# sanje2v/DualSuperResLearningForSemSeg

Hardware: AMD Instinct MI355X
Metric: stage-3 train images/sec at 256x512->512x1024 (higher is better)
Workload: dtype f32; 1 GPU; DSRL stage 3 (ResNet-101 OS16 + ASPP + SSSR/SISR decoders + FA loss), full train step, random-init weights, 256x512 input -> 512x1024 logits; global_batch=8, per_gpu_batch=8, parallelism=dp1, optimizer=SGD m0.9 wd5e-4 lr0.006

## Files before the change

dualsuperreslearningforsemseg_amd/_lib.py:

```python
import ctypes as C
import os

import torch

_HERE = os.path.dirname(os.path.abspath(__file__))
LIB_PATH = os.path.join(_HERE, 'libdsrl_hip.so')

fp = C.c_void_p
i32 = C.c_int
i64 = C.c_int64
u64 = C.c_uint64
u32 = C.c_uint32
f32 = C.c_float
sz = C.c_size_t
stream_t = C.c_void_p

_conv_shape = [i32] * 10


class WgradProblem(C.Structure):
    _fields_ = [('x', C.c_void_p), ('dy', C.c_void_p), ('dw', C.c_void_p)] + [(n, C.c_int32) for n in
                ('ldx', 'lddy', 'N', 'H', 'W', 'C', 'K', 'R', 'S', 'stride', 'pad', 'dil')] + [('x_amax', C.c_void_p), ('dy_amax', C.c_void_p)]


PROTOTYPES = {
    'dsrl_version': (i32, []),
    'dsrl_last_error': (C.c_char_p, []),
    'dsrl_device_check': (i32, [C.POINTER(i32)]),
    'dsrl_conv2d_fwd_workspace_bytes': (sz, _conv_shape),
    'dsrl_conv2d_fwd': (i32, [fp, i32, fp, fp, fp, i32] + _conv_shape + [fp, sz, stream_t]),
    'dsrl_conv2d_fwd_stats_parts': (i32, _conv_shape),
    'dsrl_conv2d_fwd_stats': (i32, [fp, i32, fp, fp, fp, i32] + _conv_shape + [fp, sz, fp, i32, stream_t]),
    'dsrl_conv2d_dgrad_workspace_bytes': (sz, _conv_shape),
    'dsrl_conv2d_transposed_filter_floats': (sz, [i32] * 4),
    'dsrl_conv2d_transpose_filter': (i32, [fp, fp, i32, i32, i32, i32, stream_t]),
    'dsrl_conv2d_transpose_filters_batched': (i32, [fp, i32, i64, stream_t]),
    'dsrl_conv2d_filters_amax_segment_floats': (i32, []),
    'dsrl_conv2d_filters_amax_batched': (i32, [fp, i64, stream_t]),
    'dsrl_conv2d_dgrad': (i32, [fp, i32, fp, fp, fp, i32] + _conv_shape + [fp, sz, stream_t]),
    'dsrl_conv2d_dgrad_stats_parts': (i32, _conv_shape),
    'dsrl_conv2d_dgrad_bnstats': (i32, [fp, i32, fp, fp, fp, i32] + _conv_shape + [fp, sz, fp, i32, fp, i32, fp, fp, i32, fp, i32, i32, stream_t]),
    'dsrl_conv2d_dgrad_accumulate': (i32, [fp, i32, fp, fp, fp, i32] + _conv_shape + [fp, sz, stream_t]),
    'dsrl_conv2d_wgrad_workspace_bytes': (sz, _conv_shape),
    'dsrl_conv2d_wgrad': (i32, [fp, i32, fp, i32, fp] + _conv_shape + [fp, sz, stream_t]),
    'dsrl_conv2d_wgrad_group_table_bytes': (sz, [i32]),
    'dsrl_conv2d_wgrad_group_workspace_bytes': (sz, [fp, i32]),
    'dsrl_conv2d_wgrad_group_plan': (i32, [fp, i32, fp, sz, fp, fp, sz]),
    'dsrl_conv2d_wgrad_group_launch': (i32, [fp, fp, stream_t]),
    'dsrl_amax': (i32, [fp, i32, i64, i32, fp, stream_t]),
    'dsrl_conv2d_fwd_amax': (i32, [fp, i32, fp, fp, fp, fp, fp, fp, i32] + _conv_shape + [fp, sz, fp, i32, stream_t]),
    'dsrl_conv2d_dgrad_amax': (i32, [fp, i32, fp, fp, fp, fp, fp, fp, i32] + _conv_shape + [fp, sz, fp, i32, fp, i32, fp, fp, i32, fp, i32, i32, stream_t]),
    'dsrl_conv2d_split_filters_batched': (i32, [fp, i32, i64, stream_t]),
    'dsrl_planes_lo_offset': (sz, [i64]),
    'dsrl_planes_bytes': (sz, [i64, i32]),
    'dsrl_split_planes': (i32, [fp, i32, i64, i32, fp, fp, i32, stream_t]),
    'dsrl_conv2d_filter_planes_batched': (i32, [fp, i32, i64, stream_t]),
    'dsrl_conv2d_fwd_planes': (i32, [fp, i32, fp, fp, fp, fp, fp, fp, fp, fp, i32] + _conv_shape + [fp, sz, fp, i32, stream_t]),
    'dsrl_conv2d_dgrad_planes': (i32, [fp, i32, fp, fp, fp, fp, fp, fp, fp, fp, i32] + _conv_shape + [fp, sz, fp, i32, fp, i32, fp, fp, i32, fp, i32, i32, stream_t]),
    'dsrl_conv2d_dgrad_planes_drop': (i32, [fp, i32, fp, fp, fp, fp, fp, fp, fp, fp, i32] + _conv_shape + [fp, sz, fp, i32, fp, i32, fp, fp, i32, f32, fp, i32, i32, stream_t]),
    'dsrl_conv2d_wgrad_amax': (i32, [fp, i32, fp, fp, i32, fp, fp] + _conv_shape + [fp, sz, stream_t]),
    'dsrl_conv_precision': (i32, [i32]),
    'dsrl_conv2d_inbounds_macs': (i64, _conv_shape),
    'dsrl_conv2d_rowfold_fwd_workspace_bytes': (sz, [i32] * 9),
    'dsrl_conv2d_rowfold_fwd': (i32, [fp, i32, fp, fp, fp, i32] + [i32] * 9 + [i64, fp, sz, stream_t]),
    'dsrl_conv2d_rowfold_wgrad_workspace_bytes': (sz, [i32] * 9),
    'dsrl_conv2d_rowfold_wgrad': (i32, [fp, i32, fp, i32, fp] + [i32] * 9 + [i64, fp, sz, stream_t]),
    'dsrl_pad_image_nhwc': (i32, [fp, i64, i64, i64, i64, fp] + [i32] * 9 + [stream_t]),
    'dsrl_colsum_workspace_bytes': (sz, [i64, i32]),
    'dsrl_colsum': (i32, [fp, i32, i64, i32, fp, fp, sz, stream_t]),
    'dsrl_bn_workspace_bytes': (sz, [i64, i32]),
# ... 122 lines not shown
```

dualsuperreslearningforsemseg_amd/command_handlers/train_or_resume.py:

```python
import glob
import os
from datetime import datetime

import torch as t
import torch.distributed as dist

from .. import functional as HF
from .. import settings
from ..ddp import FlatParams
from ..models import DSRL
from ..models.losses import FALoss


def isCUDAdevice(device):
    return device.casefold() == 'gpu'


def polynomial_lr(base_lr, end_lr, epoch, max_decay_steps, power):
    if epoch <= 0:
        return base_lr
    return (base_lr - end_lr) * ((1. - epoch / max_decay_steps) ** power) + end_lr


class SyntheticCityscapes:
# ... 139 lines not shown

    def _set_hyper(self, hp):
        vals = (float(hp[0]), float(hp[1]), float(hp[2]), 1.0 / self.flat.world)
        if vals != self._hyper_vals:
            self._hyper_host.copy_(t.tensor(vals, dtype=t.float32))
            self.hyper.copy_(self._hyper_host, non_blocking=True)
            self._hyper_vals = vals

    def _graph_key(self, input_image, input_org, target):
        return (tuple(input_image.shape), tuple(input_org.shape), tuple(target.shape), HF.get_conv_precision(), HF.overlap_wgrad)

    def _capture(self, key, input_image, input_org, target, hp):
        c = _CapturedStep()
        c.img, c.org, c.tgt = input_image.clone(), input_org.clone(), target.clone()
        bns = [m for m in self.model.modules() if isinstance(m, t.nn.modules.batchnorm._BatchNorm)]
        before = [getattr(m, '_dsrl_batches', 0) for m in bns]
        step_before = HF._rng_state['step']
        c.graph = t.cuda.CUDAGraph()
        overlap_was = HF.overlap_wgrad
        HF.overlap_wgrad = False
        c.keep = HF.graph_keepalive = []
        HF.capture_host, HF.capture_host_off = t.empty(2 << 20, dtype=t.uint8, pin_memory=True), 0
        c.keep.append(HF.capture_host)
        if HF.f16_mode():
            c.keep.append(HF.amax_pin(self.flat.device))
        c.graph_b, c.ready = None, []
        mode = 'thread_local'
        try:
            if self.split:
                with t.cuda.graph(c.graph, capture_error_mode=mode):
                    c.outs, c.vals, cuts = self._phase_a(c.img, c.org, c.tgt, True, True, True)
                c.ready = self.flat.ready_chunks()
                c.graph_b = t.cuda.CUDAGraph()
                with t.cuda.graph(c.graph_b, pool=c.graph.pool(), capture_error_mode=mode):
                    self._phase_b(cuts)
                del cuts
            else:
                with t.cuda.graph(c.graph, capture_error_mode=mode):
                    c.outs, c.vals, _ = self._phase_a(c.img, c.org, c.tgt, True, True, False)
                    self._finish(hp, True)
        finally:
            HF.overlap_wgrad = overlap_was
            HF.graph_keepalive = None
            HF.capture_host = None
        HF._rng_state['step'] = step_before
        c.bns = [m for m, n in zip(bns, before) if getattr(m, '_dsrl_batches', 0) != n]
        for m, n in zip(bns, before):
            if hasattr(m, '_dsrl_batches'):
                m._dsrl_batches = n
        self._graphs[key] = c
        return c

    def _capture_or_fall_back(self, key, input_image, input_org, target, hp):
        import sys
        bns = [m for m in self.model.modules() if isinstance(m, t.nn.modules.batchnorm._BatchNorm)]
        before = [getattr(m, '_dsrl_batches', 0) for m in bns]
        step_before, overlap_was = HF._rng_state['step'], HF.overlap_wgrad
        try:
            return self._capture(key, input_image, input_org, target, hp)
        except Exception as e:
            print(f'[dsrl] hipGraph capture failed ({type(e).__name__}: {str(e)[:200]}); this TrainStep continues with eager launches', file=sys.stderr, flush=True)
            self.use_graph = False
            HF.overlap_wgrad, HF.graph_keepalive, HF.capture_host, HF.wgrad_queue = overlap_was, None, None, None
            HF._rng_state['step'] = step_before
            for m, n in zip(bns, before):
                if hasattr(m, '_dsrl_batches'):
                    m._dsrl_batches = n
            try:
                t.cuda.set_stream(t.cuda.default_stream(self.flat.device))
                t.cuda.synchronize(self.flat.device)
            except Exception:
                pass
            return None

    def _replay(self, c, input_image, input_org, target):
        flat = self.flat
        for dst, src in ((c.img, input_image), (c.org, input_org), (c.tgt, target)):
            if dst.data_ptr() != src.data_ptr():
                dst.copy_(src, non_blocking=True)
        ev = [t.cuda.Event(enable_timing=True) for _ in range(4)] if (self.time_collectives and flat.world > 1) else None
        if flat.world > 1:
            if ev:
                ev[0].record()
            flat.sync_buffers()
            if ev:
                ev[1].record()
# ... 254 lines not shown
```

dualsuperreslearningforsemseg_amd/csrc/conv_common.h:

```cpp
#pragma once
#include "common.h"

namespace dsrl {

using f32x16 = __attribute__((ext_vector_type(16))) float;
using bf16x8 = __attribute__((ext_vector_type(8))) __bf16;
using bf16x4 = __attribute__((ext_vector_type(4))) __bf16;
using f16x8 = __attribute__((ext_vector_type(8))) _Float16;
using f16x4 = __attribute__((ext_vector_type(4))) _Float16;

template <bool F16> struct Plane;
template <> struct Plane<false> {
    using v4 = bf16x4; using v8 = bf16x8;
    static __device__ __forceinline__ v4 cvt(const float* r) { return v4{(__bf16)r[0], (__bf16)r[1], (__bf16)r[2], (__bf16)r[3]}; }
    static __device__ __forceinline__ void residual(float* r, v4 t) {
#pragma unroll
        for (int e = 0; e < 4; ++e) r[e] -= (float)t[e];
    }
    static __device__ __forceinline__ f32x16 mfma(v8 a, v8 b, f32x16 c) { return __builtin_amdgcn_mfma_f32_32x32x16_bf16(a, b, c, 0, 0, 0); }
};
__device__ __forceinline__ float f16_resid_lo(unsigned t, float r) { float d; asm("v_fma_mix_f32 %0, %1, -1.0, %2 op_sel:[0,0,0] op_sel_hi:[1,0,0]" : "=v"(d) : "v"(t), "v"(r)); return d; }
__device__ __forceinline__ float f16_resid_hi(unsigned t, float r) { float d; asm("v_fma_mix_f32 %0, %1, -1.0, %2 op_sel:[1,0,0] op_sel_hi:[1,0,0]" : "=v"(d) : "v"(t), "v"(r)); return d; }
template <> struct Plane<true> {
    using v4 = f16x4; using v8 = f16x8;
// ... 67 lines not shown
    const u32x4 v = __builtin_amdgcn_raw_buffer_load_b128(r, (int)off, 0, 0);
    return make_float4(__uint_as_float(v.x), __uint_as_float(v.y), __uint_as_float(v.z), __uint_as_float(v.w));
}

struct WgradArgs {
    const float* x; const float* dy; float* dw;
    int ldx, lddy;
    int N, H, W, C, K, R, S, Ho, Wo, stride, pad, dil;
    long long P;
    unsigned x_bytes, dy_bytes;
    int ctiles;
    int psplits;
    long long slab;
    int taps[64]; int ntaps;
    int xcd_remap;
    int kctiles;
    unsigned mHW, sHW, mW, sW;
    int kg;
    int nblocks;
    float* dw_final;
    int rblocks;
    const unsigned* amax_dy; const unsigned* amax_x;
    int no_ident;
};

bool wgrad3_eligible(int N, int H, int W, int C, int K, int R, int S, int stride, int pad, int dil, int npl, bool f16);
void wgrad3_tile(int& bm, int& bn);
int launch_wgrad3(const WgradArgs& a, int npl, hipStream_t st);
int launch_wgrad3_group(const WgradArgs* table, const int* starts, int nprob, int grid, int npl, int dil, hipStream_t st);

bool planes_cfg_supported(int cfg, int kg);
int launch_planes_igemm(const ConvArgs& a, int cfg, bool dgrad, hipStream_t st);
bool sk_supported(int cfg, int kg, int npl, bool f16, bool w_split);
size_t sk_lds_bytes();
int launch_sk_igemm(const ConvArgs& a, bool dgrad, bool str1, int npl, hipStream_t st);
__host__ __device__ inline long long planes_lo_offset(long long elems) { return (elems * 2 + 255) / 256 * 256; }

}
```

dualsuperreslearningforsemseg_amd/csrc/conv_igemm.hip:

```cpp
#include "common.h"
#include "conv_common.h"
#include <algorithm>
#include <atomic>
#include <stdlib.h>
#include <string.h>
#include <mutex>
#include <vector>

namespace dsrl {

static std::atomic<int> g_conv_precision{-1};
constexpr int BK = 32;
constexpr int LDS_LD = 36;

template <int MR, int NR, int WGM, int WGN, bool DGRAD, int MINW = 2, bool = false>
__global__ __launch_bounds__(256, MINW) void conv_igemm_f32_kernel(const ConvArgs a) {
    constexpr int BM = 32 * MR * WGM, BN = 32 * NR * WGN;
    constexpr int A_IT = BM / 32, B_IT = BN / 32;
    extern __shared__ __attribute__((aligned(16))) float smem[];

    const int tid = threadIdx.x;
    const int lane = tid & 63;
    const int wave = __builtin_amdgcn_readfirstlane(tid >> 6);
    const int wm = wave / WGN, wn = wave % WGN;
// ... 848 lines not shown
                for (int j = 0; j < NR; ++j)
#pragma unroll
                    for (int e4 = 0; e4 < 4; ++e4) {
                        const float4 v = red[((g - 1) * NQ + (i * NR + j) * 4 + e4) * 256 + tid];
                        acc[i][j][4 * e4] += v.x; acc[i][j][4 * e4 + 1] += v.y; acc[i][j][4 * e4 + 2] += v.z; acc[i][j][4 * e4 + 3] += v.w;
                    }
    }

    float* out = a.dw + (a.psplits > 1 ? (long long)zsplit * a.slab : 0ll);
    const int RS = a.R * a.S;
    const int col = lane & 31, rq = (lane >> 5) * 4;
    const int sh_out = -(sh_a + sh_b);
#pragma unroll
    for (int j = 0; j < NR; ++j) {
        const int c = c0 + (wn * NR + j) * 32 + col;
        if (c >= a.C) continue;
#pragma unroll
        for (int i = 0; i < MR; ++i) {
            const int kb = k0 + (wm * MR + i) * 32 + rq;
#pragma unroll
            for (int e = 0; e < 16; ++e) {
                const int k = kb + (e & 3) + 8 * (e >> 2);
                if (k < a.K) out[((long long)k * RS + tap) * a.C + c] = F16 ? __builtin_ldexpf(acc[i][j][e], sh_out) : acc[i][j][e];
            }
        }
    }
}

template <int MR, int NR, int WGM, int WGN, int NPL, int KG = 1, bool F16 = false>
__global__ __launch_bounds__(256 * KG, KG == 1 ? 2 : 1) void conv_wgrad_split_kernel(const WgradArgs a) {
    wgrad_split_body<MR, NR, WGM, WGN, NPL, KG, F16>(a, (int)blockIdx.x);
}

template <int MR, int NR, int WGM, int WGN, int NPL, bool F16 = false>
__global__ __launch_bounds__(256, 2) void conv_wgrad_group_kernel(const WgradArgs* __restrict__ table, const int* __restrict__ starts, int nprob) {
    const int b = (int)blockIdx.x;
    int lo = 0, hi = nprob - 1;
    while (lo < hi) {
        const int mid = (lo + hi + 1) >> 1;
        if (starts[mid] <= b) lo = mid; else hi = mid - 1;
    }
    lo = __builtin_amdgcn_readfirstlane(lo);
    const WgradArgs& a = table[lo];
    const int local = b - starts[lo];
    if (local >= a.nblocks) return;
    wgrad_split_body<MR, NR, WGM, WGN, NPL, 1, F16>(a, local);
// ... 909 lines not shown
}
extern "C" int dsrl_conv2d_wgrad_amax(const float* x, int ldx, const uint32_t* x_amax, const float* dy, int lddy, const uint32_t* dy_amax, float* dw,
                                      int N, int H, int W, int C, int K, int R, int S, int stride, int pad, int dil,
                                      void* ws, size_t ws_bytes, dsrl_stream_t stream) {
    return wgrad_impl(x, ldx, dy, lddy, dw, N, H, W, C, K, R, S, stride, pad, dil, ws, ws_bytes, stream, x_amax, dy_amax);
}


namespace dsrl {
constexpr unsigned kGroupMagic = 0x44535247u;
constexpr int kGroupMaxProblems = 512, kGroupMaxLaunches = kNumCfg + 2;
constexpr int kCfgW3 = kNumCfg;
struct GroupLaunch { int cfg, first, count, grid; double flops, bytes; };
struct GroupHeader {
    unsigned magic; int n, nlaunch, npl, f16;
    GroupLaunch launch[kGroupMaxLaunches];
    int rgrid;
    long long args_off, starts_off, rstarts_off, used_bytes;
};
static size_t group_table_bytes(int n) {
    return align_up(sizeof(GroupHeader), 256) + align_up((size_t)n * sizeof(WgradArgs), 256) + 2 * align_up((size_t)(n + 1) * sizeof(int), 256);
}
static int group_target_px() { return std::max(256, knob("DSRL_WGRAD_GROUP_PX", 4096)); }
struct GroupItem { WgradArgs a; TileCfg cfg; int bm, bn; double cost, flops, bytes; size_t slab_bytes; };
static int group_psplits(long long P, int w3_px = 0) {
    const long long chunks = ceil_div(P, 32);
    if (w3_px > 0) {
        const int forced3 = knob("DSRL_FORCE_PSPLITS", 0), px = w3_px;
        long long sp3 = forced3 > 0 ? forced3 : (P + px / 2) / px;
        sp3 = std::max<long long>(1, std::min<long long>(sp3, std::max<long long>(1, chunks / 8)));
        return (int)std::min<long long>(sp3, 256);
    }
    const int forced = knob("DSRL_FORCE_PSPLITS", 0);
    long long sp = forced > 0 ? forced : (P + group_target_px() / 2) / group_target_px();
    sp = std::max<long long>(1, std::min<long long>(sp, std::max<long long>(1, chunks / 4)));
    return (int)std::min<long long>(sp, 256);
}
static int w3_group_px(const dsrl_wgrad_problem*, int, int) { return std::max(256, knob("DSRL_WGRAD3_PX", 2048)); }
static int group_item(const dsrl_wgrad_problem& q, int npl, GroupItem& it, const int* w3_px) {
    const int N = q.N, H = q.H, W = q.W, C = q.C, K = q.K, R = q.R, S = q.S, stride = q.stride, pad = q.pad, dil = q.dil;
    if (int e = check_conv(q.x, q.dy, q.dw, N, H, W, C, K, R, S, stride, pad, dil)) return e;
    DSRL_REQUIRE(C % 4 == 0 && q.ldx % 4 == 0 && q.lddy % 4 == 0 && q.lddy >= pad4(K) && ((uintptr_t)q.x % 16) == 0 && ((uintptr_t)q.dy % 16) == 0 && ((uintptr_t)q.dw % 16) == 0,
                 DSRL_E_UNSUPPORTED, "conv2d_wgrad_group: C (%d), ldx (%d), lddy (%d) must be multiples of 4 (lddy >= K rounded up to 4), pointers 16-byte aligned", C, q.ldx, q.lddy);
    const WgPlan p = plan_wgrad(N, H, W, C, K, R, S, stride, pad, dil);
    DSRL_REQUIRE(p.P < (1ll << 31), DSRL_E_UNSUPPORTED, "conv2d_wgrad_group: more than 2^31 output pixels");
    WgradArgs a{};
    a.x = q.x; a.dy = q.dy; a.ldx = q.ldx; a.lddy = q.lddy; a.N = N; a.H = H; a.W = W; a.C = C; a.K = K; a.R = R; a.S = S; a.Ho = p.Ho; a.Wo = p.Wo;
    a.stride = stride; a.pad = pad; a.dil = dil; a.P = p.P; a.ctiles = p.ctiles; a.slab = (long long)K * R * S * C;
    const long long xb = span_bytes((long long)N * H * W, q.ldx, C), db = span_bytes(p.P, q.lddy, pad4(K));
    DSRL_REQUIRE_31(xb, "conv2d_wgrad_group(x)"); DSRL_REQUIRE_31(db, "conv2d_wgrad_group(dy)");
    a.x_bytes = (unsigned)xb; a.dy_bytes = (unsigned)db; a.no_ident = wgrad_no_ident();
    a.ntaps = p.tl.n;
    for (int i = 0; i < p.tl.n; ++i) a.taps[i] = p.tl.taps[i];
    a.psplits = group_psplits(p.P, p.w3 ? w3_px[dil - 1] : 0);
    a.kg = 1; a.kctiles = p.ktiles * p.ctiles; a.xcd_remap = knob("DSRL_XCD_REMAP", 1);
    a.nblocks = p.w3 ? a.kctiles * a.psplits : a.kctiles * a.ntaps * a.psplits;
    a.dw_final = q.dw; a.dw = q.dw;
    a.rblocks = a.psplits > 1 ? (int)ceil_div((long long)K * a.ntaps * (C / 4), 1024) : 0;
    make_magic(a.Ho * a.Wo, a.mHW, a.sHW);
    make_magic(a.Wo, a.mW, a.sW);
    DSRL_REQUIRE(!conv_f16() || (q.x_amax != nullptr && q.dy_amax != nullptr), DSRL_E_BADARG,
                 "conv2d_wgrad_group: the f16x3 arithmetic needs x_amax / dy_amax of every problem (dsrl_amax measures a tensor)");
    a.amax_x = q.x_amax; a.amax_dy = q.dy_amax;
    it.a = a; it.cfg = p.w3 ? (TileCfg)(kCfgW3 + dil - 1) : p.cfg; it.bm = p.bm; it.bn = p.bn;
    it.cost = (double)p.P / a.psplits * p.bm * p.bn;
    it.flops = 2.0 * (double)dsrl_conv2d_inbounds_macs(N, H, W, C, K, R, S, stride, pad, dil);
    it.bytes = 4.0 * ((double)N * H * W * C + (double)K * R * S * C + (double)p.P * K);
    it.slab_bytes = a.psplits > 1 ? align_up((size_t)a.psplits * a.slab * sizeof(float), 256) : 0;
    (void)npl;
    return DSRL_OK;
}
}

extern "C" size_t dsrl_conv2d_wgrad_group_table_bytes(int n) { return n > 0 ? group_table_bytes(n) : 0; }

extern "C" size_t dsrl_conv2d_wgrad_group_workspace_bytes(const dsrl_wgrad_problem* problems, int n) {
    if (!problems || n <= 0) return 0;
    size_t total = 0;
    const int w3_px[2] = {dsrl::w3_group_px(problems, n, 1), dsrl::w3_group_px(problems, n, 2)};
    for (int i = 0; i < n; ++i) {
        const dsrl_wgrad_problem& q = problems[i];
        if (q.N <= 0 || q.H <= 0 || q.W <= 0 || q.C <= 0 || q.K <= 0 || q.R <= 0 || q.S <= 0 || q.stride <= 0 || q.dil <= 0 || q.pad < 0) continue;
        if (out_size(q.H, q.R, q.stride, q.pad, q.dil) <= 0 || out_size(q.W, q.S, q.stride, q.pad, q.dil) <= 0) continue;
        const long long P = (long long)q.N * out_size(q.H, q.R, q.stride, q.pad, q.dil) * out_size(q.W, q.S, q.stride, q.pad, q.dil);
        const bool w3 = out_size(q.H, q.R, q.stride, q.pad, q.dil) == q.H && plan_wgrad(q.N, q.H, q.W, q.C, q.K, q.R, q.S, q.stride, q.pad, q.dil).w3;
        const int sp = dsrl::group_psplits(P, w3 ? w3_px[q.dil - 1] : 0);
        if (sp > 1) total += align_up((size_t)sp * q.K * q.R * q.S * q.C * sizeof(float), 256);
    }
    return total;
}

extern "C" int dsrl_conv2d_wgrad_group_plan(const dsrl_wgrad_problem* problems, int n, void* host_table, size_t table_bytes, const void* dev_table,
                                            void* ws, size_t ws_bytes) {
    DSRL_REQUIRE(problems && host_table && dev_table && n > 0 && n <= kGroupMaxProblems, DSRL_E_BADARG, "conv2d_wgrad_group_plan: bad arguments (n=%d, at most %d problems)", n, kGroupMaxProblems);
    DSRL_REQUIRE(table_bytes >= group_table_bytes(n), DSRL_E_WORKSPACE, "conv2d_wgrad_group_plan: table %zu < %zu bytes", table_bytes, group_table_bytes(n));
    DSRL_REQUIRE(((uintptr_t)dev_table % 16) == 0 && ((uintptr_t)host_table % 16) == 0, DSRL_E_BADARG, "conv2d_wgrad_group_plan: tables must be 16-byte aligned");
    const int npl = conv_planes(PASS_WGRAD);
    DSRL_REQUIRE(npl >= 1 && npl <= 3, DSRL_E_UNSUPPORTED, "conv2d_wgrad_group_plan: the grouped launch exists for the 16-bit MFMA arithmetics only (dsrl_conv_precision 1..5)");
    std::vector<GroupItem> items((size_t)n);
    size_t need_ws = 0;
    const int w3_px[2] = {w3_group_px(problems, n, 1), w3_group_px(problems, n, 2)};
    for (int i = 0; i < n; ++i) {
        if (int e = group_item(problems[i], npl, items[(size_t)i], w3_px)) return e;
        need_ws += items[(size_t)i].slab_bytes;
    }
    DSRL_REQUIRE(ws_bytes >= need_ws && (need_ws == 0 || ws), DSRL_E_WORKSPACE, "conv2d_wgrad_group_plan: workspace %zu < %zu", ws_bytes, need_ws);
    DSRL_REQUIRE(need_ws == 0 || ((uintptr_t)ws % 16) == 0, DSRL_E_BADARG, "conv2d_wgrad_group_plan: workspace must be 16-byte aligned");
    std::stable_sort(items.begin(), items.end(), [](const GroupItem& l, const GroupItem& r) { return l.cfg != r.cfg ? l.cfg < r.cfg : l.cost > r.cost; });
    char* base = (char*)host_table;
    memset(base, 0, group_table_bytes(n));
    GroupHeader* h = (GroupHeader*)base;
    h->magic = kGroupMagic; h->n = n; h->npl = npl; h->nlaunch = 0; h->f16 = conv_f16() ? 1 : 0;
    h->args_off = (long long)align_up(sizeof(GroupHeader), 256);
    h->starts_off = h->args_off + (long long)align_up((size_t)n * sizeof(WgradArgs), 256);
    h->rstarts_off = h->starts_off + (long long)align_up((size_t)(n + 1) * sizeof(int), 256);
    h->used_bytes = (long long)group_table_bytes(n);
    WgradArgs* args = (WgradArgs*)(base + h->args_off);
    int* starts = (int*)(base + h->starts_off);
    int* rstarts = (int*)(base + h->rstarts_off);
    size_t ws_off = 0;
    int rtotal = 0;
    for (int i = 0; i < n; ++i) {
        GroupItem& it = items[(size_t)i];
        if (it.a.psplits > 1) { it.a.dw = (float*)((char*)ws + ws_off); ws_off += it.slab_bytes; }
        args[i] = it.a;
        rstarts[i] = rtotal;
        rtotal += it.a.rblocks;
        if (h->nlaunch == 0 || h->launch[h->nlaunch - 1].cfg != (int)it.cfg) {
            GroupLaunch& L = h->launch[h->nlaunch++];
            L.cfg = (int)it.cfg; L.first = i; L.count = 0; L.grid = 0; L.flops = 0; L.bytes = 0;
        }
        GroupLaunch& L = h->launch[h->nlaunch - 1];
        starts[i] = L.grid;
        L.grid += (int)align_up((size_t)it.a.nblocks, 8);
        L.count += 1; L.flops += it.flops; L.bytes += it.bytes;
    }
    rstarts[n] = rtotal;
    h->rgrid = rtotal;
    return DSRL_OK;
}

extern "C" int dsrl_conv2d_wgrad_group_launch(const void* host_table, const void* dev_table, dsrl_stream_t stream) {
    DSRL_REQUIRE(host_table && dev_table, DSRL_E_BADARG, "conv2d_wgrad_group_launch: null table");
    const GroupHeader* h = (const GroupHeader*)host_table;
    DSRL_REQUIRE(h->magic == kGroupMagic && h->n > 0 && h->nlaunch > 0 && h->nlaunch <= kGroupMaxLaunches, DSRL_E_BADARG, "conv2d_wgrad_group_launch: the host table was not written by dsrl_conv2d_wgrad_group_plan");
    hipStream_t st = (hipStream_t)stream;
    if (int e = bind_stream_device(st)) return e;
    const WgradArgs* hargs = (const WgradArgs*)((const char*)host_table + h->args_off);
    const WgradArgs* dargs = (const WgradArgs*)((const char*)dev_table + h->args_off);
    const int* dstarts = (const int*)((const char*)dev_table + h->starts_off);
    const int* drstarts = (const int*)((const char*)dev_table + h->rstarts_off);
    for (int i = 0; i < h->n; ++i) {
        const WgradArgs& a = hargs[i];
        if (a.ntaps < a.R * a.S)
            if (int e = launch_zero_fill(a.dw_final, (size_t)a.K * a.R * a.S * a.C * sizeof(float), st)) return e;
    }
    const int npl = h->npl;
    for (int l = 0; l < h->nlaunch; ++l) {
        const GroupLaunch& L = h->launch[l];
        if (L.grid <= 0) continue;
        const WgradArgs* t = dargs + L.first;
        const int* s = dstarts + L.first;
        ProfScope prof(3 * prof_arith(npl, h->f16 != 0) + 1, L.flops, L.bytes, st);
        if (L.cfg >= kCfgW3) {
            if (int e = launch_wgrad3_group(t, s, L.count, L.grid, npl, L.cfg - kCfgW3 + 1, st)) return e;
            continue;
        }
        int bm, bn; cfg_dims((TileCfg)L.cfg, bm, bn);
        const size_t lds = (size_t)2 * npl * 16 * ((bm * 2 + 64) + (bn * 2 + 64));
#define DSRL_LAUNCH_WGROUP(a_, b_, c_, d_)                                                                                         \
        if (h->f16 && npl == 1) hipLaunchKernelGGL((conv_wgrad_group_kernel<a_, b_, c_, d_, 1, true>), dim3((unsigned)L.grid), dim3(256), lds, st, t, s, L.count); \
        else if (h->f16) hipLaunchKernelGGL((conv_wgrad_group_kernel<a_, b_, c_, d_, 2, true>), dim3((unsigned)L.grid), dim3(256), lds, st, t, s, L.count); \
        else if (npl == 2) hipLaunchKernelGGL((conv_wgrad_group_kernel<a_, b_, c_, d_, 2>), dim3((unsigned)L.grid), dim3(256), lds, st, t, s, L.count); \
        else hipLaunchKernelGGL((conv_wgrad_group_kernel<a_, b_, c_, d_, 3>), dim3((unsigned)L.grid), dim3(256), lds, st, t, s, L.count);
        DSRL_CFG_SWITCH((TileCfg)L.cfg, DSRL_LAUNCH_WGROUP)
#undef DSRL_LAUNCH_WGROUP
        if (int e = launch_status("conv_wgrad_group_kernel")) return e;
    }
    if (h->rgrid > 0) {
// ... 166 lines not shown
```

dualsuperreslearningforsemseg_amd/csrc/conv_wgrad3.hip:

```cpp
#include "conv_common.h"
#include <type_traits>

namespace dsrl {

namespace {
constexpr int kW3WGM = 2, kW3WGN = 2, kW3TG = 2;
constexpr int kW3Threads = 64 * kW3WGM * kW3WGN * kW3TG;
constexpr int kW3Taps0 = 5;

template <int NPL, int HALO>
struct W3Geom {
    static constexpr int BM = 32 * kW3WGM, BN = 32 * kW3WGN, NT = kW3Threads;
    static constexpr int XW = 32 + 2 * HALO, XR = 3 * XW;
    static constexpr int A_V = BM / 4, B_V = BN / 4;
    static constexpr int A_RP = NT / A_V, B_RP = NT / B_V;
    static constexpr int A_IT = 32 / A_RP, B_IT = (XR + B_RP - 1) / B_RP;
    static constexpr int SA = BM * 2 + 64, SB = BN * 2 + 64;
    static constexpr int PLA = 32 * SA, PLB = B_IT * B_RP * SB, OFF_B = NPL * PLA, STAGE = NPL * (PLA + PLB);
    static_assert(32 % A_RP == 0 && A_IT >= 1, "dy staging passes");
};

template <int NPL, int HALO>
__device__ __forceinline__ void wgrad3_body(const WgradArgs& a, const int bid) {
    using G = W3Geom<NPL, HALO>;
// ... 151 lines not shown
            for (int ch = ch0; ch < ch1; ch += 2) {
                phase(I0{}, I5{}, S0, S1, ch + 2 < ch1 ? ch + 2 : -1);
                __syncthreads();
                if (ch + 1 >= ch1) break;
                phase(I0{}, I5{}, S1, S0, ch + 3 < ch1 ? ch + 3 : -1);
                __syncthreads();
            }
        } else {
            for (int ch = ch0; ch < ch1; ch += 2) {
                phase(I5{}, I4{}, S0, S1, ch + 2 < ch1 ? ch + 2 : -1);
                __syncthreads();
                if (ch + 1 >= ch1) break;
                phase(I5{}, I4{}, S1, S0, ch + 3 < ch1 ? ch + 3 : -1);
                __syncthreads();
            }
        }
    } else {
        sh_a = amax_shift_of(am_a); sh_b = amax_shift_of(am_b);
    }

    float* out = a.dw + (a.psplits > 1 ? (long long)zsplit * a.slab : 0ll);
    const int col = lane & 31, rq = (lane >> 5) * 4;
    const int sh_out = -(sh_a + sh_b);
    const int c = c0 + wn * 32 + col;
    if (c < a.C) {
        const int kb = k0 + wm * 32 + rq;
        const int tfirst = tgrp == 0 ? 0 : kW3Taps0, ntap = tgrp == 0 ? kW3Taps0 : 9 - kW3Taps0;
#pragma unroll
        for (int j = 0; j < kW3Taps0; ++j)
            if (j < ntap) {
#pragma unroll
                for (int e = 0; e < 16; ++e) {
                    const int k = kb + (e & 3) + 8 * (e >> 2);
                    if (k < a.K) out[((long long)k * 9 + tfirst + j) * a.C + c] = __builtin_ldexpf(acc[j][e], sh_out);
                }
            }
    }
}

template <int NPL, int HALO>
__global__ __launch_bounds__(kW3Threads, 1) void conv_wgrad3_kernel(const WgradArgs a) {
    wgrad3_body<NPL, HALO>(a, (int)blockIdx.x);
}
template <int NPL, int HALO>
__global__ __launch_bounds__(kW3Threads, 1) void conv_wgrad3_group_kernel(const WgradArgs* __restrict__ table, const int* __restrict__ starts, int nprob) {
    const int b = (int)blockIdx.x;
    int lo = 0, hi = nprob - 1;
    while (lo < hi) {
        const int mid = (lo + hi + 1) >> 1;
        if (starts[mid] <= b) lo = mid; else hi = mid - 1;
    }
    lo = __builtin_amdgcn_readfirstlane(lo);
    const WgradArgs& a = table[lo];
    const int local = b - starts[lo];
    if (local >= a.nblocks) return;
    wgrad3_body<NPL, HALO>(a, local);
}
// ... 36 lines not shown
```

dualsuperreslearningforsemseg_amd/functional.py:

```python
import ctypes
import os
import weakref

import torch

from . import _lib
from ._lib import call, knob, query, DsrlHipError

CL = torch.channels_last


_raw_stream = getattr(torch._C, '_cuda_getCurrentRawStream', None)
_raw_device = getattr(torch._C, '_cuda_getDevice', None)


def _stream():
    if _raw_stream is not None and _raw_device is not None:
        return _raw_stream(_raw_device())
    return torch.cuda.current_stream().cuda_stream


_side = {}
overlap_wgrad = knob('DSRL_OVERLAP_WGRAD', True)

# ... 135 lines not shown
    _lib.check(_lib.load().dsrl_bn_fused_barrier_timeouts(ctypes.byref(n)), 'dsrl_bn_fused_barrier_timeouts')
    return int(n.value)


def side_stream(device):
    st = _side.get(device)
    if st is None:
        st = _side[device] = torch.cuda.Stream(device=device)
    return st


def join_side_streams():
    if not _side:
        return
    cur = torch.cuda.current_stream()
    for st in _side.values():
        if st.device == cur.device:
            cur.wait_stream(st)


group_wgrad = knob('DSRL_WGRAD_GROUP', True)
graph_keepalive = None
capture_host, capture_host_off = None, 0


class WgradQueue:
    def __init__(self):
        self.items = []

    def add(self, x, ldx, dy, lddy, dw, shp, on_written=None, x_amax=None, dy_amax=None):
        self.items.append((x, ldx, dy, lddy, dw, shp, on_written, x_amax, dy_amax))

    def flush(self):
        items, self.items = self.items, []
        if not items:
            return
        n = len(items)
        probs = (_lib.WgradProblem * n)()
        for q, (x, ldx, dy, lddy, dw, shp, _, xa, dya) in zip(probs, items):
            N, H, W, Cc, K, R, S, stride, pad, dil = shp
            q.x, q.dy, q.dw = x.data_ptr(), dy.data_ptr(), dw.data_ptr()
            q.x_amax = None if xa is None else xa.data_ptr()
            q.dy_amax = None if dya is None else dya.data_ptr()
            q.ldx, q.lddy, q.N, q.H, q.W, q.C, q.K, q.R, q.S, q.stride, q.pad, q.dil = ldx, lddy, N, H, W, Cc, K, R, S, stride, pad, dil
        import ctypes
        lib = _lib.load()
        like = items[0][0]
        tbytes = int(lib.dsrl_conv2d_wgrad_group_table_bytes(n))
        ws = _ws(int(lib.dsrl_conv2d_wgrad_group_workspace_bytes(ctypes.addressof(probs), n)), like)
        if graph_keepalive is not None:
            global capture_host_off
            off = (capture_host_off + 255) & ~255
            if capture_host is None or off + tbytes > capture_host.numel():
                raise DsrlHipError('WgradQueue.flush under graph capture: the pinned table arena is missing or too small')
            host = capture_host[off:off + tbytes]
            capture_host_off = off + tbytes
        else:
            host = torch.empty(tbytes, dtype=torch.uint8, pin_memory=True)
        dev = torch.empty(tbytes, dtype=torch.uint8, device=like.device)
        call('dsrl_conv2d_wgrad_group_plan', ctypes.addressof(probs), n, host.data_ptr(), tbytes, dev.data_ptr(), ws.data_ptr(), ws.numel())
        dev.copy_(host, non_blocking=True)
        if graph_keepalive is not None:
            graph_keepalive.append(host)
        call('dsrl_conv2d_wgrad_group_launch', host.data_ptr(), dev.data_ptr(), _stream())
        for it in items:
            if it[6] is not None:
                it[6]()


wgrad_queue = None


def open_wgrad_queue():
    global wgrad_queue
    wgrad_queue = WgradQueue() if (group_wgrad and get_conv_precision() != 'fp32') else None
    return wgrad_queue


def flush_wgrad_queue(reopen=False):
    global wgrad_queue
    q, wgrad_queue = wgrad_queue, None
    if q is not None:
        q.flush()
# ... 1370 lines not shown
```

include/dsrl_hip.h:

```cpp
#ifndef DSRL_HIP_H
#define DSRL_HIP_H

#include <stddef.h>
#include <stdint.h>

#ifdef __cplusplus
extern "C" {
#endif

#define DSRL_ABI_VERSION 1

#define DSRL_OK 0
#define DSRL_E_BADARG (-1)
#define DSRL_E_UNSUPPORTED (-2)
#define DSRL_E_WORKSPACE (-3)
#define DSRL_E_LAUNCH (-4)

typedef void* dsrl_stream_t;

int dsrl_version(void);
const char* dsrl_last_error(void);
int dsrl_device_check(int* cu_count);

size_t dsrl_conv2d_fwd_workspace_bytes(int N, int H, int W, int C, int K, int R, int S, int stride, int pad, int dil);
// ... 17 lines not shown
                      void* ws, size_t ws_bytes, dsrl_stream_t stream);
int dsrl_conv2d_dgrad_stats_parts(int N, int H, int W, int C, int K, int R, int S, int stride, int pad, int dil);
int dsrl_conv2d_dgrad_bnstats(const float* dy, int lddy, const float* w, const float* wt , float* dx, int lddx,
                              int N, int H, int W, int C, int K, int R, int S, int stride, int pad, int dil,
                              void* ws, size_t ws_bytes, const float* bn_x, int bn_ldx, const float* bn_y , int bn_ldy,
                              const float* bn_mean, const float* bn_invstd, int bn_relu, float* bstats, int stats_parts,
                              int accumulate , dsrl_stream_t stream);
int dsrl_conv2d_dgrad_accumulate(const float* dy, int lddy, const float* w, const float* wt , float* dx, int lddx,
                                 int N, int H, int W, int C, int K, int R, int S, int stride, int pad, int dil,
                                 void* ws, size_t ws_bytes, dsrl_stream_t stream);
size_t dsrl_conv2d_wgrad_workspace_bytes(int N, int H, int W, int C, int K, int R, int S, int stride, int pad, int dil);
int dsrl_conv2d_wgrad(const float* x, int ldx, const float* dy, int lddy, float* dw,
                      int N, int H, int W, int C, int K, int R, int S, int stride, int pad, int dil,
                      void* ws, size_t ws_bytes, dsrl_stream_t stream);
typedef struct dsrl_wgrad_problem {
    const float* x; const float* dy; float* dw;
    int32_t ldx, lddy, N, H, W, C, K, R, S, stride, pad, dil;
    const uint32_t* x_amax; const uint32_t* dy_amax;
} dsrl_wgrad_problem;
size_t dsrl_conv2d_wgrad_group_table_bytes(int n);
size_t dsrl_conv2d_wgrad_group_workspace_bytes(const dsrl_wgrad_problem* problems, int n);
int dsrl_conv2d_wgrad_group_plan(const dsrl_wgrad_problem* problems, int n, void* host_table, size_t table_bytes, const void* dev_table,
                                 void* ws, size_t ws_bytes);
int dsrl_conv2d_wgrad_group_launch(const void* host_table, const void* dev_table, dsrl_stream_t stream);
#define DSRL_AMAX_WORDS 256
int dsrl_amax(const float* x, int ld, int64_t P, int C, uint32_t* amax, dsrl_stream_t stream);
int dsrl_conv2d_fwd_amax(const float* x, int ldx, const uint32_t* x_amax, const float* w, const uint32_t* w_amax, const void* w_split ,
                         const float* bias , float* y, int ldy, int N, int H, int W, int C, int K, int R, int S, int stride, int pad, int dil,
                         void* ws, size_t ws_bytes, float* stats , int stats_parts, dsrl_stream_t stream);
int dsrl_conv2d_dgrad_amax(const float* dy, int lddy, const uint32_t* dy_amax, const float* w, const float* wt , const uint32_t* w_amax,
                           const void* wt_split , float* dx, int lddx, int N, int H, int W, int C, int K, int R, int S, int stride, int pad, int dil,
                           void* ws, size_t ws_bytes, const float* bn_x, int bn_ldx, const float* bn_y, int bn_ldy,
                           const float* bn_mean, const float* bn_invstd, int bn_relu, float* bstats , int stats_parts, int accumulate,
                           dsrl_stream_t stream);
size_t dsrl_planes_lo_offset(int64_t elems);
size_t dsrl_planes_bytes(int64_t elems, int nplanes);
int dsrl_split_planes(const float* x, int ld, int64_t P, int C, const uint32_t* amax, void* planes, int nplanes, dsrl_stream_t stream);
int dsrl_conv2d_filter_planes_batched(const int64_t* table, int n, int64_t total_tiles, dsrl_stream_t stream);
int dsrl_conv2d_fwd_planes(const float* x, int ldx, const uint32_t* x_amax, const void* x_planes , const float* w, const uint32_t* w_amax,
                           const void* w_split , const void* w_planes , const float* bias , float* y, int ldy,
                           int N, int H, int W, int C, int K, int R, int S, int stride, int pad, int dil,
                           void* ws, size_t ws_bytes, float* stats , int stats_parts, dsrl_stream_t stream);
int dsrl_conv2d_dgrad_planes(const float* dy, int lddy, const uint32_t* dy_amax, const void* dy_planes , const float* w, const float* wt ,
                             const uint32_t* w_amax, const void* wt_split , const void* wt_planes , float* dx, int lddx,
                             int N, int H, int W, int C, int K, int R, int S, int stride, int pad, int dil,
                             void* ws, size_t ws_bytes, const float* bn_x, int bn_ldx, const float* bn_y, int bn_ldy,
// ... 180 lines not shown
```

Baseline: 493.9 images/s.

## Fuse split-K wgrad reduction into 3x3 kernel via atomic tickets; drop zero-fill

For grouped 3x3 weight-gradient launches with 2-4 pixel splits, each split now writes only its own compact tile partials. A per-tile atomic ticket lets the last-arriving block sum all partials and write the final gradient directly, so the separate reduction pass (rblocks=0) is no longer needed and the slab workspace shrinks. Pruned-tap zeroing also moves into the kernel epilogue, replacing the per-problem zero-fill memsets. The cost is extra global traffic for partial tiles, atomic synchronisation, and a ticket buffer that has to be managed across graph capture.

```diff
diff --git a/dualsuperreslearningforsemseg_amd/_lib.py b/dualsuperreslearningforsemseg_amd/_lib.py
--- a/dualsuperreslearningforsemseg_amd/_lib.py
+++ b/dualsuperreslearningforsemseg_amd/_lib.py
@@ -46,6 +46,8 @@
     'dsrl_conv2d_wgrad_group_table_bytes': (sz, [i32]),
     'dsrl_conv2d_wgrad_group_workspace_bytes': (sz, [fp, i32]),
     'dsrl_conv2d_wgrad_group_plan': (i32, [fp, i32, fp, sz, fp, fp, sz]),
+    'dsrl_conv2d_wgrad_group_ticket_bytes': (sz, [fp, i32]),
+    'dsrl_conv2d_wgrad_group_plan_tickets': (i32, [fp, i32, fp, sz, fp, fp, sz, fp, sz]),
     'dsrl_conv2d_wgrad_group_launch': (i32, [fp, fp, stream_t]),
     'dsrl_amax': (i32, [fp, i32, i64, i32, fp, stream_t]),
     'dsrl_conv2d_fwd_amax': (i32, [fp, i32, fp, fp, fp, fp, fp, fp, i32] + _conv_shape + [fp, sz, fp, i32, stream_t]),
diff --git a/dualsuperreslearningforsemseg_amd/command_handlers/train_or_resume.py b/dualsuperreslearningforsemseg_amd/command_handlers/train_or_resume.py
--- a/dualsuperreslearningforsemseg_amd/command_handlers/train_or_resume.py
+++ b/dualsuperreslearningforsemseg_amd/command_handlers/train_or_resume.py
@@ -185,6 +185,8 @@
         c.keep = HF.graph_keepalive = []
         HF.capture_host, HF.capture_host_off = t.empty(2 << 20, dtype=t.uint8, pin_memory=True), 0
         c.keep.append(HF.capture_host)
+        HF.capture_tickets, HF.capture_tickets_off = HF.new_ticket_buffer(self.flat.device), 0
+        c.keep.append(HF.capture_tickets)
         if HF.f16_mode():
             c.keep.append(HF.amax_pin(self.flat.device))
         c.graph_b, c.ready = None, []
@@ -206,6 +208,7 @@
             HF.overlap_wgrad = overlap_was
             HF.graph_keepalive = None
             HF.capture_host = None
+            HF.capture_tickets = None
         HF._rng_state['step'] = step_before
         c.bns = [m for m, n in zip(bns, before) if getattr(m, '_dsrl_batches', 0) != n]
         for m, n in zip(bns, before):
@@ -224,7 +227,7 @@
         except Exception as e:
             print(f'[dsrl] hipGraph capture failed ({type(e).__name__}: {str(e)[:200]}); this TrainStep continues with eager launches', file=sys.stderr, flush=True)
             self.use_graph = False
-            HF.overlap_wgrad, HF.graph_keepalive, HF.capture_host, HF.wgrad_queue = overlap_was, None, None, None
+            HF.overlap_wgrad, HF.graph_keepalive, HF.capture_host, HF.capture_tickets, HF.wgrad_queue = overlap_was, None, None, None, None
             HF._rng_state['step'] = step_before
             for m, n in zip(bns, before):
                 if hasattr(m, '_dsrl_batches'):
diff --git a/dualsuperreslearningforsemseg_amd/csrc/conv_common.h b/dualsuperreslearningforsemseg_amd/csrc/conv_common.h
--- a/dualsuperreslearningforsemseg_amd/csrc/conv_common.h
+++ b/dualsuperreslearningforsemseg_amd/csrc/conv_common.h
@@ -113,7 +113,10 @@
     int rblocks;
     const unsigned* amax_dy; const unsigned* amax_x;
     int no_ident;
+    unsigned* tickets; unsigned part_bytes;
+    int zero_pruned;
 };
+constexpr int kW3TileFloats = 64 * 64 * 9;
 
 bool wgrad3_eligible(int N, int H, int W, int C, int K, int R, int S, int stride, int pad, int dil, int npl, bool f16);
 void wgrad3_tile(int& bm, int& bn);
diff --git a/dualsuperreslearningforsemseg_amd/csrc/conv_igemm.hip b/dualsuperreslearningforsemseg_amd/csrc/conv_igemm.hip
--- a/dualsuperreslearningforsemseg_amd/csrc/conv_igemm.hip
+++ b/dualsuperreslearningforsemseg_amd/csrc/conv_igemm.hip
@@ -894,6 +894,29 @@
             for (int e = 0; e < 16; ++e) {
                 const int k = kb + (e & 3) + 8 * (e >> 2);
                 if (k < a.K) out[((long long)k * RS + tap) * a.C + c] = F16 ? __builtin_ldexpf(acc[i][j][e], sh_out) : acc[i][j][e];
+            }
+        }
+    }
+    if (a.zero_pruned && zsplit == 0) {
+        int u = 0;
+        for (int t = 0; t < RS; ++t) {
+            bool live = false;
+            for (int i = 0; i < a.ntaps; ++i) live |= a.taps[i] == t;
+            if (live) continue;
+            if (u++ % a.ntaps != tapi) continue;
+#pragma unroll
+            for (int j = 0; j < NR; ++j) {
+                const int c = c0 + (wn * NR + j) * 32 + col;
+                if (c >= a.C) continue;
+#pragma unroll
+                for (int i = 0; i < MR; ++i) {
+                    const int kb = k0 + (wm * MR + i) * 32 + rq;
+#pragma unroll
+                    for (int e = 0; e < 16; ++e) {
+                        const int k = kb + (e & 3) + 8 * (e >> 2);
+                        if (k < a.K) a.dw_final[((long long)k * RS + t) * a.C + c] = 0.f;
+                    }
+                }
             }
         }
     }
@@ -1849,7 +1872,15 @@
     return align_up(sizeof(GroupHeader), 256) + align_up((size_t)n * sizeof(WgradArgs), 256) + 2 * align_up((size_t)(n + 1) * sizeof(int), 256);
 }
 static int group_target_px() { return std::max(256, knob("DSRL_WGRAD_GROUP_PX", 4096)); }
-struct GroupItem { WgradArgs a; TileCfg cfg; int bm, bn; double cost, flops, bytes; size_t slab_bytes; };
+struct GroupItem { WgradArgs a; TileCfg cfg; int bm, bn; double cost, flops, bytes; size_t slab_bytes; int coop_tiles; };
+static bool group_w3_coop(bool w3, int psplits, int kctiles) {
+    return w3 && psplits >= 2 && psplits <= 4 && (long long)psplits * kctiles * kW3TileFloats * 4 < (1ll << 31) && knob("DSRL_WGRAD_COOP", 1) != 0;
+}
+static size_t group_slab_bytes(bool w3, int psplits, int K, int RS, int C, int kctiles) {
+    if (psplits <= 1) return 0;
+    const size_t per = group_w3_coop(w3, psplits, kctiles) ? (size_t)kctiles * kW3TileFloats : (size_t)K * RS * C;
+    return align_up((size_t)psplits * per * sizeof(float), 256);
+}
 static int group_psplits(long long P, int w3_px = 0) {
     const long long chunks = ceil_div(P, 32);
     if (w3_px > 0) {
@@ -1893,7 +1924,9 @@
     it.cost = (double)p.P / a.psplits * p.bm * p.bn;
     it.flops = 2.0 * (double)dsrl_conv2d_inbounds_macs(N, H, W, C, K, R, S, stride, pad, dil);
     it.bytes = 4.0 * ((double)N * H * W * C + (double)K * R * S * C + (double)p.P * K);
-    it.slab_bytes = a.psplits > 1 ? align_up((size_t)a.psplits * a.slab * sizeof(float), 256) : 0;
+    it.slab_bytes = group_slab_bytes(p.w3, a.psplits, K, R * S, C, a.kctiles);
+    it.coop_tiles = group_w3_coop(p.w3, a.psplits, a.kctiles) ? a.kctiles : 0;
+    it.a.zero_pruned = a.ntaps < R * S ? 1 : 0;
     (void)npl;
     return DSRL_OK;
 }
@@ -1910,27 +1943,52 @@
         if (q.N <= 0 || q.H <= 0 || q.W <= 0 || q.C <= 0 || q.K <= 0 || q.R <= 0 || q.S <= 0 || q.stride <= 0 || q.dil <= 0 || q.pad < 0) continue;
         if (out_size(q.H, q.R, q.stride, q.pad, q.dil) <= 0 || out_size(q.W, q.S, q.stride, q.pad, q.dil) <= 0) continue;
         const long long P = (long long)q.N * out_size(q.H, q.R, q.stride, q.pad, q.dil) * out_size(q.W, q.S, q.stride, q.pad, q.dil);
-        const bool w3 = out_size(q.H, q.R, q.stride, q.pad, q.dil) == q.H && plan_wgrad(q.N, q.H, q.W, q.C, q.K, q.R, q.S, q.stride, q.pad, q.dil).w3;
+        const WgPlan p = plan_wgrad(q.N, q.H, q.W, q.C, q.K, q.R, q.S, q.stride, q.pad, q.dil);
+        const bool w3 = out_size(q.H, q.R, q.stride, q.pad, q.dil) == q.H && p.w3;
         const int sp = dsrl::group_psplits(P, w3 ? w3_px[q.dil - 1] : 0);
-        if (sp > 1) total += align_up((size_t)sp * q.K * q.R * q.S * q.C * sizeof(float), 256);
+        total += dsrl::group_slab_bytes(w3, sp, q.K, q.R * q.S, q.C, p.ktiles * p.ctiles);
     }
     return total;
+}
+
+extern "C" size_t dsrl_conv2d_wgrad_group_ticket_bytes(const dsrl_wgrad_problem* problems, int n) {
+    if (!problems || n <= 0) return 0;
+    size_t words = 0;
+    const int w3_px[2] = {dsrl::w3_group_px(problems, n, 1), dsrl::w3_group_px(problems, n, 2)};
+    for (int i = 0; i < n; ++i) {
+        const dsrl_wgrad_problem& q = problems[i];
+        if (q.N <= 0 || q.H <= 0 || q.W <= 0 || q.C <= 0 || q.K <= 0 || q.R <= 0 || q.S <= 0 || q.stride <= 0 || q.dil <= 0 || q.pad < 0) continue;
+        if (out_size(q.H, q.R, q.stride, q.pad, q.dil) <= 0 || out_size(q.W, q.S, q.stride, q.pad, q.dil) <= 0) continue;
+        const long long P = (long long)q.N * out_size(q.H, q.R, q.stride, q.pad, q.dil) * out_size(q.W, q.S, q.stride, q.pad, q.dil);
+        const WgPlan p = plan_wgrad(q.N, q.H, q.W, q.C, q.K, q.R, q.S, q.stride, q.pad, q.dil);
+        const bool w3 = out_size(q.H, q.R, q.stride, q.pad, q.dil) == q.H && p.w3;
+        if (dsrl::group_w3_coop(w3, dsrl::group_psplits(P, w3 ? w3_px[q.dil - 1] : 0), p.ktiles * p.ctiles)) words += (size_t)p.ktiles * p.ctiles;
+    }
+    return words * sizeof(unsigned);
 }
 
 extern "C" int dsrl_conv2d_wgrad_group_plan(const dsrl_wgrad_problem* problems, int n, void* host_table, size_t table_bytes, const void* dev_table,
                                             void* ws, size_t ws_bytes) {
+    return dsrl_conv2d_wgrad_group_plan_tickets(problems, n, host_table, table_bytes, dev_table, ws, ws_bytes, nullptr, 0);
+}
+
+extern "C" int dsrl_conv2d_wgrad_group_plan_tickets(const dsrl_wgrad_problem* problems, int n, void* host_table, size_t table_bytes, const void* dev_table,
+                                                    void* ws, size_t ws_bytes, void* tickets, size_t ticket_bytes) {
     DSRL_REQUIRE(problems && host_table && dev_table && n > 0 && n <= kGroupMaxProblems, DSRL_E_BADARG, "conv2d_wgrad_group_plan: bad arguments (n=%d, at most %d problems)", n, kGroupMaxProblems);
     DSRL_REQUIRE(table_bytes >= group_table_bytes(n), DSRL_E_WORKSPACE, "conv2d_wgrad_group_plan: table %zu < %zu bytes", table_bytes, group_table_bytes(n));
     DSRL_REQUIRE(((uintptr_t)dev_table % 16) == 0 && ((uintptr_t)host_table % 16) == 0, DSRL_E_BADARG, "conv2d_wgrad_group_plan: tables must be 16-byte aligned");
     const int npl = conv_planes(PASS_WGRAD);
     DSRL_REQUIRE(npl >= 1 && npl <= 3, DSRL_E_UNSUPPORTED, "conv2d_wgrad_group_plan: the grouped launch exists for the 16-bit MFMA arithmetics only (dsrl_conv_precision 1..5)");
     std::vector<GroupItem> items((size_t)n);
-    size_t need_ws = 0;
+    size_t need_ws = 0, need_tk = 0;
     const int w3_px[2] = {w3_group_px(problems, n, 1), w3_group_px(problems, n, 2)};
     for (int i = 0; i < n; ++i) {
         if (int e = group_item(problems[i], npl, items[(size_t)i], w3_px)) return e;
         need_ws += items[(size_t)i].slab_bytes;
-    }
+        if (tickets) need_tk += (size_t)items[(size_t)i].coop_tiles * sizeof(unsigned);
+    }
+    DSRL_REQUIRE(ticket_bytes >= need_tk, DSRL_E_WORKSPACE, "conv2d_wgrad_group_plan: ticket buffer %zu < %zu bytes", ticket_bytes, need_tk);
+    DSRL_REQUIRE(need_tk == 0 || ((uintptr_t)tickets % 4) == 0, DSRL_E_BADARG, "conv2d_wgrad_group_plan: ticket buffer must be 4-byte aligned");
     DSRL_REQUIRE(ws_bytes >= need_ws && (need_ws == 0 || ws), DSRL_E_WORKSPACE, "conv2d_wgrad_group_plan: workspace %zu < %zu", ws_bytes, need_ws);
     DSRL_REQUIRE(need_ws == 0 || ((uintptr_t)ws % 16) == 0, DSRL_E_BADARG, "conv2d_wgrad_group_plan: workspace must be 16-byte aligned");
     std::stable_sort(items.begin(), items.end(), [](const GroupItem& l, const GroupItem& r) { return l.cfg != r.cfg ? l.cfg < r.cfg : l.cost > r.cost; });
@@ -1945,11 +2003,21 @@
     WgradArgs* args = (WgradArgs*)(base + h->args_off);
     int* starts = (int*)(base + h->starts_off);
     int* rstarts = (int*)(base + h->rstarts_off);
-    size_t ws_off = 0;
+    size_t ws_off = 0, tk_off = 0;
     int rtotal = 0;
     for (int i = 0; i < n; ++i) {
         GroupItem& it = items[(size_t)i];
         if (it.a.psplits > 1) { it.a.dw = (float*)((char*)ws + ws_off); ws_off += it.slab_bytes; }
+        if (tickets && it.coop_tiles > 0) {
+            const long long pb = (long long)it.a.psplits * it.coop_tiles * kW3TileFloats * (long long)sizeof(float);
+            DSRL_REQUIRE_31(pb, "conv2d_wgrad_group_plan(partial tiles)");
+            DSRL_REQUIRE((size_t)pb <= it.slab_bytes && tk_off + (size_t)it.coop_tiles <= ticket_bytes / sizeof(unsigned), DSRL_E_WORKSPACE,
+                         "conv2d_wgrad_group_plan: partial area or ticket buffer too small");
+            it.a.part_bytes = (unsigned)pb;
+            it.a.tickets = (unsigned*)tickets + tk_off;
+            tk_off += (size_t)it.coop_tiles;
+            it.a.rblocks = 0;
+        }
         args[i] = it.a;
         rstarts[i] = rtotal;
         rtotal += it.a.rblocks;
@@ -1973,15 +2041,9 @@
     DSRL_REQUIRE(h->magic == kGroupMagic && h->n > 0 && h->nlaunch > 0 && h->nlaunch <= kGroupMaxLaunches, DSRL_E_BADARG, "conv2d_wgrad_group_launch: the host table was not written by dsrl_conv2d_wgrad_group_plan");
     hipStream_t st = (hipStream_t)stream;
     if (int e = bind_stream_device(st)) return e;
-    const WgradArgs* hargs = (const WgradArgs*)((const char*)host_table + h->args_off);
     const WgradArgs* dargs = (const WgradArgs*)((const char*)dev_table + h->args_off);
     const int* dstarts = (const int*)((const char*)dev_table + h->starts_off);
     const int* drstarts = (const int*)((const char*)dev_table + h->rstarts_off);
-    for (int i = 0; i < h->n; ++i) {
-        const WgradArgs& a = hargs[i];
-        if (a.ntaps < a.R * a.S)
-            if (int e = launch_zero_fill(a.dw_final, (size_t)a.K * a.R * a.S * a.C * sizeof(float), st)) return e;
-    }
     const int npl = h->npl;
     for (int l = 0; l < h->nlaunch; ++l) {
         const GroupLaunch& L = h->launch[l];
diff --git a/dualsuperreslearningforsemseg_amd/csrc/conv_wgrad3.hip b/dualsuperreslearningforsemseg_amd/csrc/conv_wgrad3.hip
--- a/dualsuperreslearningforsemseg_amd/csrc/conv_wgrad3.hip
+++ b/dualsuperreslearningforsemseg_amd/csrc/conv_wgrad3.hip
@@ -197,17 +197,101 @@
     float* out = a.dw + (a.psplits > 1 ? (long long)zsplit * a.slab : 0ll);
     const int col = lane & 31, rq = (lane >> 5) * 4;
     const int sh_out = -(sh_a + sh_b);
+    const int tfirst = tgrp == 0 ? 0 : kW3Taps0, ntap = tgrp == 0 ? kW3Taps0 : 9 - kW3Taps0;
+#pragma unroll
+    for (int j = 0; j < kW3Taps0; ++j)
+#pragma unroll
+        for (int e = 0; e < 16; ++e) acc[j][e] = __builtin_ldexpf(acc[j][e], sh_out);
+
+    if (a.tickets != nullptr) {
+        constexpr int kSC1 = 16;
+        constexpr unsigned kTileBytes = (unsigned)kW3TileFloats * 4u;
+        const int nz = a.psplits;
+        const __amdgpu_buffer_rsrc_t pr = __builtin_amdgcn_make_buffer_rsrc((void*)a.dw, 0, (int)a.part_bytes, 0x00020000);
+        const unsigned tile_off = (unsigned)kc * kTileBytes, zstride = (unsigned)a.kctiles * kTileBytes;
+        auto voff = [&](int v) -> unsigned { return v < 16 ? (unsigned)(v * kW3Threads + tid) * 16u : (unsigned)(16 * kW3Threads + (v - 16) * (kW3Threads / 2) + tid) * 16u; };
+#pragma unroll
+        for (int j = 0; j < kW3Taps0; ++j)
+            if (j < ntap) {
+#pragma unroll
+                for (int q = 0; q < 4; ++q) {
+                    const u32x4 v = {__float_as_uint(acc[j][4 * q]), __float_as_uint(acc[j][4 * q + 1]), __float_as_uint(acc[j][4 * q + 2]), __float_as_uint(acc[j][4 * q + 3])};
+                    __builtin_amdgcn_raw_buffer_store_b128(v, pr, (int)(tile_off + (unsigned)zsplit * zstride + voff(4 * j + q)), 0, kSC1);
+                }
+            }
+        asm volatile("s_waitcnt vmcnt(0)" ::: "memory");
+        volatile int* const last_flag = reinterpret_cast<volatile int*>(smem);
+        __syncthreads();
+        if (threadIdx.x == 0) {
+            unsigned* tk = a.tickets + kc;
+            const unsigned old = __hip_atomic_fetch_add(tk, 1u, __ATOMIC_RELAXED, __HIP_MEMORY_SCOPE_AGENT);
+            const int last = old == (unsigned)(nz - 1);
+            if (last) __hip_atomic_store(tk, 0u, __ATOMIC_RELAXED, __HIP_MEMORY_SCOPE_AGENT);
+            *last_flag = last;
+        }
+        __syncthreads();
+        if (!*last_flag) return;
+        if (nz == 2) {
+            const unsigned ooff = tile_off + (unsigned)(1 - zsplit) * zstride;
+            u32x4 in[kW3Taps0][4];
+#pragma unroll
+            for (int j = 0; j < kW3Taps0; ++j)
+                if (j < ntap) {
+#pragma unroll
+                    for (int q = 0; q < 4; ++q) in[j][q] = __builtin_amdgcn_raw_buffer_load_b128(pr, (int)(ooff + voff(4 * j + q)), 0, kSC1);
+                }
+#pragma unroll
+            for (int j = 0; j < kW3Taps0; ++j)
+                if (j < ntap) {
+#pragma unroll
+                    for (int e = 0; e < 16; ++e) {
+                        const float o = __uint_as_float(in[j][e >> 2][e & 3]);
+                        float s = 0.f;
+                        s += zsplit == 0 ? acc[j][e] : o;
+                        s += zsplit == 0 ? o : acc[j][e];
+                        acc[j][e] = s;
+                    }
+                }
+        } else
+#pragma unroll
+        for (int j = 0; j < kW3Taps0; ++j)
+            if (j < ntap) {
+                u32x4 in[4][4];
+#pragma unroll
+                for (int z = 0; z < 4; ++z) {
+                    const unsigned zoff = (z < nz && z != zsplit) ? (unsigned)z * zstride : kOOB;
+#pragma unroll
+                    for (int q = 0; q < 4; ++q)
+                        in[z][q] = __builtin_amdgcn_raw_buffer_load_b128(pr, (int)__builtin_elementwise_add_sat(zoff, tile_off + voff(4 * j + q)), 0, kSC1);
+                }
+#pragma unroll
+                for (int e = 0; e < 16; ++e) {
+                    float p[4];
+#pragma unroll
+                    for (int z = 0; z < 4; ++z) p[z] = z == zsplit ? acc[j][e] : __uint_as_float(in[z][e >> 2][e & 3]);
+                    float s = 0.f;
+                    if (nz == 4) {
+                        s += (p[0] + p[1]) + (p[2] + p[3]);
+                    } else {
+                        s += p[0]; s += p[1];
+                        if (nz > 2) s += p[2];
+                    }
+                    acc[j][e] = s;
+                }
+            }
+        out = a.dw_final;
+    }
+
     const int c = c0 + wn * 32 + col;
     if (c < a.C) {
         const int kb = k0 + wm * 32 + rq;
-        const int tfirst = tgrp == 0 ? 0 : kW3Taps0, ntap = tgrp == 0 ? kW3Taps0 : 9 - kW3Taps0;
 #pragma unroll
         for (int j = 0; j < kW3Taps0; ++j)
             if (j < ntap) {
 #pragma unroll
                 for (int e = 0; e < 16; ++e) {
                     const int k = kb + (e & 3) + 8 * (e >> 2);
-                    if (k < a.K) out[((long long)k * 9 + tfirst + j) * a.C + c] = __builtin_ldexpf(acc[j][e], sh_out);
+                    if (k < a.K) out[((long long)k * 9 + tfirst + j) * a.C + c] = acc[j][e];
                 }
             }
     }
diff --git a/dualsuperreslearningforsemseg_amd/functional.py b/dualsuperreslearningforsemseg_amd/functional.py
--- a/dualsuperreslearningforsemseg_amd/functional.py
+++ b/dualsuperreslearningforsemseg_amd/functional.py
@@ -181,6 +181,30 @@
 group_wgrad = knob('DSRL_WGRAD_GROUP', True)
 graph_keepalive = None
 capture_host, capture_host_off = None, 0
+_TICKET_BYTES = 256 << 10
+_tickets = {}
+capture_tickets, capture_tickets_off = None, 0
+
+
+def new_ticket_buffer(device, nbytes=_TICKET_BYTES):
+    return torch.zeros(max(int(nbytes), 256), dtype=torch.uint8, device=device)
+
+
+def _ticket_buffer(nbytes, like):
+    global capture_tickets_off
+    if nbytes <= 0:
+        return None
+    if graph_keepalive is not None:
+        off = (capture_tickets_off + 255) & ~255
+        if capture_tickets is not None and capture_tickets.device == like.device and off + nbytes <= capture_tickets.numel():
+            capture_tickets_off = off + nbytes
+            return capture_tickets[off:off + nbytes]
+        return new_ticket_buffer(like.device, nbytes)
+    key = (like.device, _stream())
+    buf = _tickets.get(key)
+    if buf is None or buf.numel() < nbytes:
+        buf = _tickets[key] = new_ticket_buffer(like.device, max(nbytes, _TICKET_BYTES))
+    return buf
 
 
 class WgradQueue:
@@ -207,6 +231,7 @@
         like = items[0][0]
         tbytes = int(lib.dsrl_conv2d_wgrad_group_table_bytes(n))
         ws = _ws(int(lib.dsrl_conv2d_wgrad_group_workspace_bytes(ctypes.addressof(probs), n)), like)
+        tk = _ticket_buffer(int(lib.dsrl_conv2d_wgrad_group_ticket_bytes(ctypes.addressof(probs), n)), like)
         if graph_keepalive is not None:
             global capture_host_off
             off = (capture_host_off + 255) & ~255
@@ -217,7 +242,8 @@
         else:
             host = torch.empty(tbytes, dtype=torch.uint8, pin_memory=True)
         dev = torch.empty(tbytes, dtype=torch.uint8, device=like.device)
-        call('dsrl_conv2d_wgrad_group_plan', ctypes.addressof(probs), n, host.data_ptr(), tbytes, dev.data_ptr(), ws.data_ptr(), ws.numel())
+        call('dsrl_conv2d_wgrad_group_plan_tickets', ctypes.addressof(probs), n, host.data_ptr(), tbytes, dev.data_ptr(), ws.data_ptr(), ws.numel(),
+             None if tk is None else tk.data_ptr(), 0 if tk is None else tk.numel())
         dev.copy_(host, non_blocking=True)
         if graph_keepalive is not None:
             graph_keepalive.append(host)
diff --git a/include/dsrl_hip.h b/include/dsrl_hip.h
--- a/include/dsrl_hip.h
+++ b/include/dsrl_hip.h
@@ -63,6 +63,9 @@
 size_t dsrl_conv2d_wgrad_group_workspace_bytes(const dsrl_wgrad_problem* problems, int n);
 int dsrl_conv2d_wgrad_group_plan(const dsrl_wgrad_problem* problems, int n, void* host_table, size_t table_bytes, const void* dev_table,
                                  void* ws, size_t ws_bytes);
+size_t dsrl_conv2d_wgrad_group_ticket_bytes(const dsrl_wgrad_problem* problems, int n);
+int dsrl_conv2d_wgrad_group_plan_tickets(const dsrl_wgrad_problem* problems, int n, void* host_table, size_t table_bytes, const void* dev_table,
+                                         void* ws, size_t ws_bytes, void* tickets, size_t ticket_bytes);
 int dsrl_conv2d_wgrad_group_launch(const void* host_table, const void* dev_table, dsrl_stream_t stream);
 #define DSRL_AMAX_WORDS 256
 int dsrl_amax(const float* x, int ld, int64_t P, int C, uint32_t* amax, dsrl_stream_t stream);
```

Result: no change. 495.4 images/s (median of 6 runs) (+0.3%).
